# NoliNobdon/TriStage-RAG

Measured on AMD Instinct MI355X. Metric: end-to-end queries/sec @10Mx768 corpus (stage-1 exact top-k, pre-encoded HBM-resident queries), higher is better.
Workload: dtype f16; 1 GPU; synthetic 10000000x768 f16 corpus, batch-64 queries, stage-1 exact top-1000, row-sharded over 1 GPU(s); rows=10000000, dim=768, batch=64, k=1000, submission=batches enqueued back to back (async), verified by finish() in the timed region, max_candidates_per_query=6027

## Files before the change

### tristage-rag_amd/csrc/ts_scan.hip

```cpp
#include "ts_scan_dev.h"
#include "ts_linear_dev.h"
#include <stdlib.h>

template <int DT, int QH, int MODE>
__global__ __launch_bounds__(SCAN_THREADS) void scan_kernel(ScanParams p) {
  extern __shared__ __attribute__((aligned(16))) unsigned char smem[];
  u32x4* qlds = reinterpret_cast<u32x4*>(smem);
  const int tid = threadIdx.x;
  const int lane = tid & 63;
  const int wave = tid >> 6;
  const int kg = p.kg;

  const int64_t nwaves = (int64_t)gridDim.x * SCAN_WAVES;
  int64_t w = (int64_t)blockIdx.x * SCAN_WAVES + wave;
  const bool active = w < p.nwork;
  const u32x4* base = reinterpret_cast<const u32x4*>(p.corpus) + lane;
  const size_t blk_units = (size_t)kg * 64;
  int64_t blk = active ? p.blk0 + w * p.blk_stride : p.blk0;
  const u32x4* cur = base + (size_t)blk * blk_units;
  u32x4 ring[TS_RING];
  if (active) {
#pragma unroll
    for (int i = 0; i < TS_RING; ++i) ring[i] = stream_load(cur + (size_t)i * 64);
  }

  {
    const u32x4* src = reinterpret_cast<const u32x4*>(p.qimg);
    const int units = kg * QH * 64;
    for (int i0 = tid; i0 < units; i0 += 8 * SCAN_THREADS) {
      u32x4 t[8];
#pragma unroll
      for (int j = 0; j < 8; ++j) {
        const int i = i0 + j * SCAN_THREADS;
        t[j] = (i < units) ? src[i] : u32x4{0, 0, 0, 0};
      }
#pragma unroll
      for (int j = 0; j < 8; ++j) {
        const int i = i0 + j * SCAN_THREADS;
        if (i < units) qlds[i] = t[j];
      }
    }
  }
  StageLds* st = reinterpret_cast<StageLds*>(smem + (size_t)kg * QH * 1024);
  if constexpr (MODE == SCAN_FILTER) {
    if (tid == 0) st->cnt = 0;
  }
  __syncthreads();

  if (active) {

  float tau[QH];
  if constexpr (MODE == SCAN_FILTER) {
#pragma unroll
    for (int hq = 0; hq < QH; ++hq) tau[hq] = p.tau[hq * 32 + (lane & 31)];
  }

  const u32x4* ql = qlds + lane;

  while (true) {
    const int64_t wn = w + nwaves;
    const bool has_next = wn < p.nwork;
    const int64_t blkn = has_next ? (p.blk0 + wn * p.blk_stride) : blk;
    const u32x4* nxt = base + (size_t)blkn * blk_units;

    f32x16 acc[QH];
#pragma unroll
    for (int hq = 0; hq < QH; ++hq)
#pragma unroll
      for (int r = 0; r < 16; ++r) acc[hq][r] = 0.f;

    int g0 = 0;
    for (; g0 < kg - TS_RING; g0 += TS_RING) {
#pragma unroll
      for (int i = 0; i < TS_RING; ++i) {
#pragma unroll
        for (int hq = 0; hq < QH; ++hq) {
#if defined(TS_TUNING) && defined(DBG_NO_LDS)
          const u32x4 b = ring[(i + 1) % TS_RING];
#else
          const u32x4 b = ql[(size_t)((g0 + i) * QH + hq) * 64];
#endif
          mma_group<DT>(acc[hq], ring[i], b);
        }
        ring[i] = stream_load(cur + (size_t)(g0 + i + TS_RING) * 64);
        __builtin_amdgcn_sched_barrier(0);
      }
    }
#pragma unroll
    for (int i = 0; i < TS_RING; ++i) {
#pragma unroll
      for (int hq = 0; hq < QH; ++hq) {
#if defined(TS_TUNING) && defined(DBG_NO_LDS)
        const u32x4 b = ring[(i + 1) % TS_RING];
#else
        const u32x4 b = ql[(size_t)((g0 + i) * QH + hq) * 64];
#endif
        mma_group<DT>(acc[hq], ring[i], b);
      }
      ring[i] = stream_load(nxt + (size_t)i * 64);
      __builtin_amdgcn_sched_barrier(0);
    }

    if constexpr (MODE == SCAN_DENSE)
      epilogue_dense<QH>(p, acc, w, blk, lane);
    else
      epilogue_filter<QH>(p, st, acc, tau, blk, lane);

    if (!has_next) break;
    w = wn;
    blk = blkn;
    cur = nxt;
  }
  }
  if constexpr (MODE == SCAN_FILTER) flush_stage(p, st, tid);
}

typedef const uint32_t __attribute__((address_space(4)))* ts_sgpr_u32p;
typedef const int32_t __attribute__((address_space(4)))* ts_sgpr_i32p;

template <int DT, int QH>
__global__ __launch_bounds__(SCAN_THREADS) void scan_masked_kernel(MaskedScanParams p) {
  extern __shared__ __attribute__((aligned(16))) unsigned char smem[];
  u32x4* qlds = reinterpret_cast<u32x4*>(smem);
  const int tid = threadIdx.x;
  const int lane = tid & 63;
  const int wave = __builtin_amdgcn_readfirstlane(tid >> 6);
  const int kg = p.kg;

  const int64_t nwaves = (int64_t)gridDim.x * SCAN_WAVES;
  int64_t w = (int64_t)blockIdx.x * SCAN_WAVES + wave;
  const int64_t nwork = (int64_t)*(ts_sgpr_u32p)p.nlive;
  const bool active = w < nwork;
  const u32x4* base = reinterpret_cast<const u32x4*>(p.corpus) + lane;
  const size_t blk_units = (size_t)kg * 64;
  int64_t blk = active ? (int64_t)((ts_sgpr_i32p)p.live)[w] : 0;
  const u32x4* cur = base + (size_t)blk * blk_units;
  u32x4 ring[TS_RING];
  if (active) {
#pragma unroll
    for (int i = 0; i < TS_RING; ++i) ring[i] = stream_load(cur + (size_t)i * 64);
  }

  {
    const u32x4* src = reinterpret_cast<const u32x4*>(p.qimg);
    const int units = kg * QH * 64;
    for (int i0 = tid; i0 < units; i0 += 8 * SCAN_THREADS) {
      u32x4 t[8];
#pragma unroll
      for (int j = 0; j < 8; ++j) {
        const int i = i0 + j * SCAN_THREADS;
        t[j] = (i < units) ? src[i] : u32x4{0, 0, 0, 0};
      }
#pragma unroll
      for (int j = 0; j < 8; ++j) {
        const int i = i0 + j * SCAN_THREADS;
        if (i < units) qlds[i] = t[j];
      }
    }
  }
  StageLds* st = reinterpret_cast<StageLds*>(smem + (size_t)kg * QH * 1024);
  if (tid == 0) st->cnt = 0;
  __syncthreads();

  if (active) {

  float tau[QH];
  const uint32_t* mrow[QH];
  int64_t mstep[QH];
  uint32_t mor[QH], mw[QH];
#pragma unroll
  for (int hq = 0; hq < QH; ++hq) {
    tau[hq] = p.tau[hq * 32 + (lane & 31)];
    const int32_t qm = p.qmask[hq * 32 + (lane & 31)];
    mrow[hq] = p.allow_bits + (qm < 0 ? 0 : (int64_t)qm * p.allow_words);
    mstep[hq] = qm < 0 ? 0 : 1;
    mor[hq] = qm < 0 ? ~0u : 0u;
    mw[hq] = mrow[hq][blk * mstep[hq]] | mor[hq];
  }

  const u32x4* ql = qlds + lane;

  while (true) {
    const int64_t wn = w + nwaves;
    const bool has_next = wn < nwork;
    const int64_t blkn = has_next ? (int64_t)((ts_sgpr_i32p)p.live)[wn] : blk;
    const u32x4* nxt = base + (size_t)blkn * blk_units;

    f32x16 acc[QH];
#pragma unroll
    for (int hq = 0; hq < QH; ++hq)
#pragma unroll
      for (int r = 0; r < 16; ++r) acc[hq][r] = 0.f;

    int g0 = 0;
    for (; g0 < kg - TS_RING; g0 += TS_RING) {
#pragma unroll
      for (int i = 0; i < TS_RING; ++i) {
#pragma unroll
        for (int hq = 0; hq < QH; ++hq) {
          const u32x4 b = ql[(size_t)((g0 + i) * QH + hq) * 64];
          mma_group<DT>(acc[hq], ring[i], b);
        }
        ring[i] = stream_load(cur + (size_t)(g0 + i + TS_RING) * 64);
        __builtin_amdgcn_sched_barrier(0);
      }
    }
    uint32_t mwn[QH];
#pragma unroll
    for (int hq = 0; hq < QH; ++hq) mwn[hq] = mrow[hq][blkn * mstep[hq]];
#pragma unroll
    for (int i = 0; i < TS_RING; ++i) {
#pragma unroll
      for (int hq = 0; hq < QH; ++hq) {
        const u32x4 b = ql[(size_t)((g0 + i) * QH + hq) * 64];
        mma_group<DT>(acc[hq], ring[i], b);
      }
      ring[i] = stream_load(nxt + (size_t)i * 64);
      __builtin_amdgcn_sched_barrier(0);
    }

    epilogue_filter<QH, StageLds, true>(p, st, acc, tau, blk, lane, mw);

    if (!has_next) break;
    w = wn;
    blk = blkn;
    cur = nxt;
#pragma unroll
    for (int hq = 0; hq < QH; ++hq) mw[hq] = mwn[hq] | mor[hq];
  }
  }
  flush_stage(p, st, tid);
}

struct StageMultiHdr {
  uint32_t cnt;
  uint32_t pad[3];
  uint32_t qcnt[TS_MAX_GROUPS * 32];
  uint32_t qbase[TS_MAX_GROUPS * 32];
  uint32_t qoff[TS_MAX_GROUPS * 32];
};
static_assert(SCAN_WAVES <= 8 && TS_MAX_GROUPS * 32 <= 128, "survivor key fields");
#define TS_MULTI_MAX_ITERS (1 << 17)
#define TS_MULTI_MIN_STAGE 1024u
#define TS_MULTI_MAX_STAGE 4096u

template <int G, class T, int N>
__device__ __forceinline__ T pick_group(const T (&a)[N], int g) {
  T r = a[0];
#pragma unroll
  for (int i = 1; i < G; ++i) r = (g == i) ? a[i] : r;
  return r;
}

template <int G, int QB, bool TOMB, class P, class H>
__device__ __forceinline__ void epilogue_multi(const P& p, H* st, float* sscore,
                                               uint32_t* skey, const f32x16 (&acc)[G], const float (&tau)[G],
                                               int64_t blk, uint32_t keyhi, int lane) {
#if defined(TS_TUNING) && defined(DBG_EPILOGUE_MASKS)
  bool hit = false;
#pragma unroll
  for (int hq = 0; hq < G; ++hq) hit |= (acc_max(acc[hq]) >= tau[hq]);
  if (__builtin_amdgcn_ballot_w64(hit) == 0ull) return;
  const int64_t row_base = blk * TS_ROWS_PER_BLOCK;
  const int j = lane & 31;
#pragma unroll
  for (int hq = 0; hq < G; ++hq) {
    uint32_t mask = 0;
#pragma unroll
    for (int r = 0; r < 16; ++r) {
      const bool ok = (acc[hq][r] >= tau[hq]) && (row_base + acc_row(r, lane) < p.ntotal);
      mask |= ok ? (1u << r) : 0u;
    }
    if (mask) {
      uint32_t slot = atomicAdd(&st->cnt, (uint32_t)__builtin_popcount(mask));
#pragma unroll
      for (int r = 0; r < 16; ++r) {
        if (mask & (1u << r)) {
          if (slot < p.stage_cap) {
            sscore[slot] = acc[hq][r];
            skey[slot] = keyhi | ((uint32_t)acc_row(r, lane) << QB) | (uint32_t)(hq * 32 + j);
          } else {
            if constexpr (TOMB) {
              atomicMax(&p.gcnt[hq][j], p.cand_cap + 1u);
            } else {
              const uint32_t g = atomicAdd(&p.gcnt[hq][j], 1u);
              if (g < p.cand_cap) {
                p.gscore[hq][(size_t)j * p.cand_cap + g] = acc[hq][r];
                p.gid[hq][(size_t)j * p.cand_cap + g] = (int32_t)(row_base + acc_row(r, lane));
              }
            }
          }
          ++slot;
        }
      }
    }
  }
#else
  uint64_t gm[G], any = 0;
#pragma unroll
  for (int hq = 0; hq < G; ++hq) {
    gm[hq] = __builtin_amdgcn_ballot_w64(acc_max(acc[hq]) >= tau[hq]);
    any |= gm[hq];
  }
  if (any == 0ull) return;
  const int64_t row_base = blk * TS_ROWS_PER_BLOCK;
  const bool partial = row_base + TS_ROWS_PER_BLOCK > p.ntotal;
  const int rows_left = (int)(p.ntotal - row_base);
#pragma unroll
  for (int hq = 0; hq < G; ++hq) {
    if (gm[hq] == 0ull) continue;
#pragma unroll
    for (int r = 0; r < 16; ++r) {
      const bool ok = acc[hq][r] >= tau[hq];
      if (__builtin_expect(__builtin_amdgcn_ballot_w64(ok) == 0ull, 1)) continue;
      if (!ok) continue;
      int ln = lane;
      __asm__ volatile("" : "+v"(ln));
      const int row = acc_row(r, ln), j = ln & 31;
      if (!partial || row < rows_left) {
        const uint32_t slot = atomicAdd(&st->cnt, 1u);
        if (slot < p.stage_cap) {
          sscore[slot] = acc[hq][r];
          skey[slot] = keyhi | ((uint32_t)row << QB) | (uint32_t)(hq * 32 + j);
        } else {
          if constexpr (TOMB) {
            atomicMax(&p.gcnt[hq][j], p.cand_cap + 1u);
          } else {
            const uint32_t g = atomicAdd(&p.gcnt[hq][j], 1u);
            if (g < p.cand_cap) {
              p.gscore[hq][(size_t)j * p.cand_cap + g] = acc[hq][r];
              p.gid[hq][(size_t)j * p.cand_cap + g] = (int32_t)(row_base + row);
            }
          }
        }
      }
    }
  }
#endif
}

template <bool TOMB, class P>
__device__ __forceinline__ bool tomb_live(const P& p, int64_t row) {
  if constexpr (TOMB) return (p.live[row >> 5] >> (row & 31)) & 1u;
  return true;
}

template <int DT, int G, bool TOMB>
__global__ __launch_bounds__(SCAN_THREADS) void scan_multi_kernel(
    std::conditional_t<TOMB, MultiTombParams, MultiScanParams> p) {
  extern __shared__ __attribute__((aligned(16))) unsigned char smem[];
  u32x4* qlds = reinterpret_cast<u32x4*>(smem);
  const int tid = threadIdx.x;
  const int lane = tid & 63;
  const int wave = __builtin_amdgcn_readfirstlane(tid >> 6);
  const int kg = p.kg;

  const int64_t nwaves = (int64_t)gridDim.x * SCAN_WAVES;
  int64_t w = (int64_t)blockIdx.x * SCAN_WAVES + wave;
  const bool active = w < p.nwork;
  const u32x4* base = reinterpret_cast<const u32x4*>(p.corpus) + lane;
  const size_t blk_units = (size_t)kg * 64;
  int64_t blk = active ? p.blk0 + w * p.blk_stride : p.blk0;
  const u32x4* cur = base + (size_t)blk * blk_units;
  u32x4 ring[TS_RING];
  if (active) {
#pragma unroll
    for (int i = 0; i < TS_RING; ++i) ring[i] = stream_load(cur + (size_t)i * 64);
  }

  {
    const int units = kg * G * 64;
    for (int i0 = tid; i0 < units; i0 += 8 * SCAN_THREADS) {
      u32x4 t[8];
#pragma unroll
      for (int jj = 0; jj < 8; ++jj) {
        const int i = i0 + jj * SCAN_THREADS;
        t[jj] = u32x4{0, 0, 0, 0};
        if (i < units) {
          const int u = i >> 6, gk = u / G, g = u - gk * G;
          const u32x4* src = reinterpret_cast<const u32x4*>(pick_group<G>(p.gimg, g));
          t[jj] = src[(size_t)(gk * pick_group<G>(p.gqh, g) + pick_group<G>(p.ghalf, g)) * 64 + (i & 63)];
        }
      }
#pragma unroll
      for (int jj = 0; jj < 8; ++jj) {
        const int i = i0 + jj * SCAN_THREADS;
        if (i < units) qlds[i] = t[jj];
      }
    }
  }
  StageMultiHdr* st = reinterpret_cast<StageMultiHdr*>(smem + (size_t)kg * G * 1024);
  float* sscore = reinterpret_cast<float*>(st + 1);
  uint32_t* skey = reinterpret_cast<uint32_t*>(sscore + p.stage_cap);
  if (tid == 0) st->cnt = 0;
  __syncthreads();

  if (active) {

  float tau[G];
#pragma unroll
  for (int hq = 0; hq < G; ++hq) tau[hq] = p.gtau[hq][lane & 31];

  const u32x4* ql = qlds + lane;
  uint32_t keyhi = (uint32_t)wave << 12;

  while (true) {
    const int64_t wn = w + nwaves;
    const bool has_next = wn < p.nwork;
    const int64_t blkn = has_next ? (p.blk0 + wn * p.blk_stride) : blk;
    const u32x4* nxt = base + (size_t)blkn * blk_units;

    f32x16 acc[G];
#pragma unroll
    for (int hq = 0; hq < G; ++hq)
#pragma unroll
      for (int r = 0; r < 16; ++r) acc[hq][r] = 0.f;

    int g0 = 0;
    for (; g0 < kg - TS_RING; g0 += TS_RING) {
#pragma unroll
      for (int i = 0; i < TS_RING; ++i) {
#pragma unroll
        for (int hq = 0; hq < G; ++hq) {
          const u32x4 b = ql[(size_t)((g0 + i) * G + hq) * 64];
          mma_group<DT>(acc[hq], ring[i], b);
        }
        ring[i] = stream_load(cur + (size_t)(g0 + i + TS_RING) * 64);
        __builtin_amdgcn_sched_barrier(0);
      }
    }
#pragma unroll
    for (int i = 0; i < TS_RING; ++i) {
#pragma unroll
      for (int hq = 0; hq < G; ++hq) {
        const u32x4 b = ql[(size_t)((g0 + i) * G + hq) * 64];
        mma_group<DT>(acc[hq], ring[i], b);
      }
      ring[i] = stream_load(nxt + (size_t)i * 64);
      __builtin_amdgcn_sched_barrier(0);
    }

    epilogue_multi<G, 7, TOMB>(p, st, sscore, skey, acc, tau, blk, keyhi, lane);

    if (!has_next) break;
    w = wn;
    blk = blkn;
    cur = nxt;
    keyhi += 1u << 15;
  }
  }

  __syncthreads();
  const uint32_t n = st->cnt < p.stage_cap ? st->cnt : p.stage_cap;
  if (n == 0) return;
  if (tid < G * 32) { st->qcnt[tid] = 0; st->qoff[tid] = 0; }
  __syncthreads();
  auto key_row = [&](uint32_t key) {
    const int64_t wi = (int64_t)blockIdx.x * SCAN_WAVES + ((key >> 12) & 7u) + (int64_t)(key >> 15) * nwaves;
    return (p.blk0 + wi * p.blk_stride) * TS_ROWS_PER_BLOCK + ((key >> 7) & 31u);
  };
  for (uint32_t e = tid; e < n; e += SCAN_THREADS) {
    if constexpr (TOMB)
      if (!tomb_live<TOMB>(p, key_row(skey[e]))) continue;
    atomicAdd(&st->qcnt[skey[e] & 127u], 1u);
  }
  __syncthreads();
  if (tid < G * 32 && st->qcnt[tid] > 0)
    st->qbase[tid] = atomicAdd(pick_group<G>(p.gcnt, tid >> 5) + (tid & 31), st->qcnt[tid]);
  __syncthreads();
  for (uint32_t e = tid; e < n; e += SCAN_THREADS) {
    const uint32_t key = skey[e];
    if constexpr (TOMB)
      if (!tomb_live<TOMB>(p, key_row(key))) continue;
    const uint32_t q = key & 127u;
    const uint32_t slot = st->qbase[q] + atomicAdd(&st->qoff[q], 1u);
    if (slot < p.cand_cap) {
      const int g = (int)(q >> 5);
      const size_t at = (size_t)(q & 31u) * p.cand_cap + slot;
      const int64_t wi = (int64_t)blockIdx.x * SCAN_WAVES + ((key >> 12) & 7u) + (int64_t)(key >> 15) * nwaves;
      pick_group<G>(p.gscore, g)[at] = sscore[e];
      pick_group<G>(p.gid, g)[at] = (int32_t)((p.blk0 + wi * p.blk_stride) * TS_ROWS_PER_BLOCK + ((key >> 7) & 31u));
    }
  }
}

int ts_scan_multi_groups(const TsLayout& L) {
  if (L.dtype != TS_F16 && L.dtype != TS_BF16) return 0;
  for (int G = TS_MAX_GROUPS; G >= 1; --G)
    if (ts_scan_multi_stage_cap(L, G) > 0) return G;
  return 0;
}

uint32_t ts_scan_multi_stage_cap(const TsLayout& L, int G) {
  const size_t fixed = (size_t)L.kg * G * 1024 + sizeof(StageMultiHdr);
  if (G < 1 || G > TS_MAX_GROUPS || fixed + 8 * (size_t)TS_MULTI_MIN_STAGE > 160 * 1024) return 0;
  return (uint32_t)std::min<size_t>(TS_MULTI_MAX_STAGE, (160 * 1024 - fixed) / 8);
}

bool ts_scan_multi_fits(int64_t nblk, int num_cus) {
  const int64_t want = (nblk + SCAN_WAVES - 1) / SCAN_WAVES;
  const int64_t grid = std::max<int64_t>(1, std::min<int64_t>(want, num_cus));
  const int64_t nwaves = grid * SCAN_WAVES;
  return (nblk + nwaves - 1) / nwaves <= TS_MULTI_MAX_ITERS;
}

template <int DT, int G, class P = MultiScanParams>
static int launch_scan_multi_t(const TsLayout& L, const P& p, int num_cus, hipStream_t stream) {
  const size_t lds = (size_t)L.kg * G * 1024 + sizeof(StageMultiHdr) + 8 * (size_t)p.stage_cap;
  void (*kern)(P) = scan_multi_kernel<DT, G, std::is_same<P, MultiTombParams>::value>;
  static TsDeviceOnce lds_attr;
  TS_CHECK(ts_allow_max_lds(lds_attr, reinterpret_cast<const void*>(kern)));
  const int64_t want = (p.nwork + SCAN_WAVES - 1) / SCAN_WAVES;
  int grid = (int)(want < num_cus ? want : num_cus);
  if (grid < 1) grid = 1;
  hipLaunchKernelGGL(kern, dim3(grid), dim3(SCAN_THREADS), lds, stream, p);
  TS_HIP(hipGetLastError());
  return TS_OK;
}

template <class P>
static int launch_scan_multi_any(const TsLayout& L, int G, const P& p, int num_cus, hipStream_t stream) {
  if (p.nwork <= 0) return TS_OK;
  if (p.stage_cap == 0 || p.stage_cap > ts_scan_multi_stage_cap(L, G) || !ts_scan_multi_fits(p.nwork, num_cus)) {
    ts_set_error("multi-group scan: %d groups do not fit at dimension %d", G, L.dim);
    return TS_ERR_UNSUPPORTED;
  }
#define TS_MULTI_G(DT)                                                      \
  switch (G) {                                                              \
    case 1: return launch_scan_multi_t<DT, 1, P>(L, p, num_cus, stream);    \
    case 2: return launch_scan_multi_t<DT, 2, P>(L, p, num_cus, stream);    \
    case 3: return launch_scan_multi_t<DT, 3, P>(L, p, num_cus, stream);    \
    case 4: return launch_scan_multi_t<DT, 4, P>(L, p, num_cus, stream);    \
  }
  switch (L.dtype) {
    case TS_F16: TS_MULTI_G(TS_F16); break;
    case TS_BF16: TS_MULTI_G(TS_BF16); break;
  }
#undef TS_MULTI_G
  ts_set_error("multi-group scan: bad dtype %d or group count %d", L.dtype, G);
  return TS_ERR_UNSUPPORTED;
}

int ts_launch_scan_multi(const TsLayout& L, int G, const MultiScanParams& p, int num_cus, hipStream_t stream) {
  return launch_scan_multi_any(L, G, p, num_cus, stream);
}

int ts_launch_scan_multi_tomb(const TsLayout& L, int G, const MultiTombParams& p, int num_cus, hipStream_t stream) {
  return launch_scan_multi_any(L, G, p, num_cus, stream);
}

struct StageWideHdr {
  uint32_t cnt;
  uint32_t pad[3];
  uint32_t qcnt[TS_MAX_WIDE_GROUPS * 32];
  uint32_t qbase[TS_MAX_WIDE_GROUPS * 32];
  uint32_t qoff[TS_MAX_WIDE_GROUPS * 32];
};
static_assert(SCAN_WAVES <= 8 && TS_MAX_WIDE_GROUPS * 32 <= 256, "wide survivor key fields");
static_assert(SCAN_THREADS == TS_RING * 64, "a window is G units per thread");
#define TS_WIDE_GROUPS 6
#define TS_WIDE_MAX_ITERS (1 << 16)
#define TS_WIDE_MIN_STAGE 4096u
#define TS_WIDE_MAX_STAGE 8192u

template <int N, int I = 0, class F>
__device__ __forceinline__ void ts_static_for(F&& f) {
  if constexpr (I < N) {
    f(std::integral_constant<int, I>{});
    ts_static_for<N, I + 1>(f);
  }
}

template <int I>
__device__ __forceinline__ void wide_ring_load(u32x4& r, uint32_t loff, const unsigned char* fill) {
#if defined(TS_TUNING) && defined(DBG_NO_MFMA)
  r = stream_load(reinterpret_cast<const u32x4*>(fill + loff + I * 1024));
#else
  __asm__ volatile("s_nop 4\n\tglobal_load_dwordx4 %0, %1, %2 offset:%3 nt"
                   : "=v"(r) : "v"(loff), "s"(fill + (I / 4) * 4096), "i"((I % 4) * 1024) : "memory");
#endif
}

#if defined(TS_TUNING) && defined(WIDE_TRACE)
#define WIDE_TRACE_ROW 10
__device__ uint32_t wide_trace_buf[256 * SCAN_WAVES * WIDE_TRACE_ROW];
extern "C" int ts_debug_wide_trace(uint32_t* out) {
  return hipMemcpyFromSymbol(out, HIP_SYMBOL(wide_trace_buf), sizeof(wide_trace_buf)) == hipSuccess ? 0 : -2;
}
#define WIDE_TRACE_BEGIN()                                              \
  uint32_t wt_sum[6] = {0, 0, 0, 0, 0, 0};                              \
  const uint32_t wt_c0 = (uint32_t)__builtin_readcyclecounter();        \
  const uint32_t wt_t0 = (uint32_t)__builtin_amdgcn_s_memrealtime();    \
  uint32_t wt_last = wt_t0
#define WIDE_STAMP(k)                                                   \
  do {                                                                  \
    __builtin_amdgcn_sched_barrier(0);                                  \
    const uint32_t now_ = (uint32_t)__builtin_amdgcn_s_memrealtime();   \
    wt_sum[k] += now_ - wt_last;                                        \
    wt_last = now_;                                                     \
    __builtin_amdgcn_sched_barrier(0);                                  \
  } while (0)
#define WIDE_STAMP_READS(k)                                             \
  do {                                                                  \
    __builtin_amdgcn_sched_barrier(0);                                  \
    __builtin_amdgcn_s_waitcnt(0xC07F);                 \
    WIDE_STAMP(k);                                                      \
  } while (0)
#define WIDE_TRACE_END(nwindows)                                                                     \
  do {                                                                                               \
    if (lane == 0 && blockIdx.x < 256) {                                                             \
      uint32_t* row_ = wide_trace_buf + ((size_t)blockIdx.x * SCAN_WAVES + wave) * WIDE_TRACE_ROW;   \
      for (int k_ = 0; k_ < 6; ++k_) row_[k_] = wt_sum[k_];                                          \
      row_[6] = (uint32_t)__builtin_amdgcn_s_memrealtime() - wt_t0;                                  \
      row_[7] = (uint32_t)__builtin_readcyclecounter() - wt_c0;                                      \
      row_[8] = (uint32_t)(nwindows);                                                                \
    }                                                                                                \
  } while (0)
#else
#define WIDE_TRACE_BEGIN() do { } while (0)
#define WIDE_STAMP(k) do { } while (0)
#define WIDE_STAMP_READS(k) do { } while (0)
#define WIDE_TRACE_END(nwindows) do { } while (0)
#endif

#if defined(TS_TUNING) && defined(DBG_WIDE_STAGGER)
#define TS_WIDE_STAGGER DBG_WIDE_STAGGER
#else
#define TS_WIDE_STAGGER (-1)
#endif
static_assert(TS_WIDE_STAGGER >= -1 && TS_WIDE_STAGGER < TS_RING - 1, "stagger slots");

template <int DT, int G, bool TOMB>
__global__ __launch_bounds__(SCAN_THREADS) void scan_wide_kernel(
    std::conditional_t<TOMB, WideTombParams, WideScanParams> p) {
  extern __shared__ __attribute__((aligned(16))) unsigned char smem[];
  constexpr int WU = G * TS_RING * 64;
  u32x4* win = reinterpret_cast<u32x4*>(smem);
  const int tid = threadIdx.x;
  const int lane = tid & 63;
  const int wave = __builtin_amdgcn_readfirstlane(tid >> 6);
  const int kg = p.kg;
  const int nwin = kg / TS_RING;

  const int64_t nwaves = (int64_t)gridDim.x * SCAN_WAVES;
  const int64_t w0 = (int64_t)blockIdx.x * SCAN_WAVES;
  int64_t w = w0 + wave;
  const bool active = w < p.nwork;
  const size_t blk_units = (size_t)kg * 64;
  int64_t blk = active ? p.blk0 + w * p.blk_stride : p.blk0;

  const int64_t my_iters = active ? (p.nwork - 1 - w) / nwaves + 1 : 0;
  const int64_t wg_iters = w0 < p.nwork ? (p.nwork - 1 - w0) / nwaves + 1 : 0;
  const int64_t tw_mine = my_iters * nwin, tw_all = wg_iters * nwin;

  const unsigned char* corpus = reinterpret_cast<const unsigned char*>(p.corpus);
  const uint32_t loff = (uint32_t)lane * 16;
  int64_t fw = w;
  const unsigned char* fill = corpus + (size_t)blk * blk_units * 16;
  const unsigned char* const fill_dead = reinterpret_cast<const unsigned char*>(p.gimg[0]);
  bool fill_done = false;
  int fwin = 0;
  auto advance_fill = [&]() {
    if (fill_done) return;
    if (++fwin < nwin) {
      fill += TS_RING * 1024;
    } else if (fw + nwaves < p.nwork) {
      fwin = 0;
      fw += nwaves;
      fill = corpus + (size_t)(p.blk0 + fw * p.blk_stride) * blk_units * 16;
    } else {
      fill_done = true;
      fill = fill_dead;
    }
  };
#if defined(TS_TUNING) && defined(DBG_WIDE_L2_RING)
  fill = fill_dead;
  fill_done = true;
#endif
  auto refill = [&](u32x4& r, auto slot) { wide_ring_load<decltype(slot)::value>(r, loff, fill); };
  auto ring_wait = [&](u32x4& r, auto slot) {
    constexpr int I = decltype(slot)::value;
    __asm__ volatile("s_waitcnt vmcnt(%1)" : "+v"(r)
                     : "i"(I <= TS_WIDE_STAGGER ? 2 * TS_RING - 1 + G - I : 2 * TS_RING - 1 + 2 * G));
  };

  const unsigned char* qsrc[G];
  int64_t qstep[G];
#pragma unroll
  for (int j = 0; j < G; ++j) {
    const int v = wave + SCAN_WAVES * j, i = v / G, g = v - i * G;
    const int gqh = pick_group<G>(p.gqh, g);
    qsrc[j] = reinterpret_cast<const unsigned char*>(pick_group<G>(p.gimg, g)) +
              (size_t)(i * gqh + pick_group<G>(p.ghalf, g)) * 1024;
    qstep[j] = (int64_t)gqh * TS_RING * 1024;
  }
  const uint32_t win_lds = (uint32_t)(uintptr_t)(__attribute__((address_space(3))) void*)(win + wave * 64);
  auto gather = [&](int wi, int b) {
#pragma unroll
    for (int j = 0; j < G; ++j) {
      const unsigned char* src = qsrc[j] + wi * qstep[j];
      const uint32_t dst = win_lds + (uint32_t)(b * WU + j * SCAN_THREADS) * 16;
      uint32_t keep;
      __asm__ volatile("s_nop 4\n\ts_mov_b32 %0, m0\n\ts_mov_b32 m0, %3\n\ts_nop 0\n\t"
                       "global_load_lds_dwordx4 %1, %2\n\ts_mov_b32 m0, %0"
                       : "=&s"(keep) : "v"(loff), "s"(src), "s"(dst) : "memory");
    }
  };

  StageWideHdr* st = reinterpret_cast<StageWideHdr*>(smem + (size_t)2 * WU * 16);
  float* sscore = reinterpret_cast<float*>(st + 1);
  uint32_t* skey = reinterpret_cast<uint32_t*>(sscore + p.stage_cap);
  if (tid == 0) st->cnt = 0;

  float tau[G];
#pragma unroll
  for (int hq = 0; hq < G; ++hq) tau[hq] = p.gtau[hq][lane & 31];
#pragma unroll
  for (int hq = 0; hq < G; ++hq) __asm__ volatile("" : "+v"(tau[hq]));
  u32x4 ring[2 * TS_RING];
  if (active) {
    ts_static_for<TS_RING>([&](auto i) { refill(ring[i], i); });
    advance_fill();
  }
  gather(0, 0);
  if (active) {
    ts_static_for<TS_RING>([&](auto i) { refill(ring[TS_RING + i], i); });
    advance_fill();
    __builtin_amdgcn_s_waitcnt(0x3F70 | TS_RING);
  } else {
    __builtin_amdgcn_s_waitcnt(0x3F70);
  }
  fs_barrier();

  uint32_t keyhi = (uint32_t)wave << 13;

  f32x16 acc[G];
#pragma unroll
  for (int hq = 0; hq < G; ++hq)
#pragma unroll
    for (int r = 0; r < 16; ++r) acc[hq][r] = 0.f;

  auto walk_barrier = [&]() {
#if defined(TS_TUNING) && defined(DBG_WIDE_NO_BARRIER)
    __builtin_amdgcn_s_waitcnt(0xC07F);
#else
    fs_barrier();
#endif
  };
  int qw = 0;
  WIDE_TRACE_BEGIN();
  auto window = [&](auto half) {
    constexpr int P = decltype(half)::value;
    const int qn = qw + 1 < nwin ? qw + 1 : 0;
    __builtin_amdgcn_s_waitcnt(0xC07F);
    const bool late = TS_WIDE_STAGGER >= 0 && wave >= SCAN_WAVES / 2;
    if (!late) gather(qn, P ^ 1);
    WIDE_STAMP(0);
    const u32x4* ql = win + P * WU + lane;
#if !(defined(TS_TUNING) && defined(DBG_WIDE_SERIAL_B))
    u32x4 bb[G];
#pragma unroll
    for (int hq = 0; hq < G; ++hq) bb[hq] = ql[hq * 64];
#endif
    WIDE_STAMP_READS(1);
    ts_static_for<TS_RING>([&](auto i) {
#if defined(TS_TUNING) && defined(DBG_WIDE_SERIAL_B)
      ring_wait(ring[P * TS_RING + i], i);
#pragma unroll
      for (int hq = 0; hq < G; ++hq) {
        const u32x4 b = ql[(i * G + hq) * 64];
        mma_group<DT>(acc[hq], ring[P * TS_RING + i], b);
      }
#else
      __builtin_amdgcn_sched_barrier(0);
      ring_wait(ring[P * TS_RING + i], i);
#pragma unroll
      for (int hq = 0; hq < G; ++hq) {
        mma_group<DT>(acc[hq], ring[P * TS_RING + i], bb[hq]);
        __builtin_amdgcn_sched_barrier(0);
        if constexpr (decltype(i)::value + 1 < TS_RING) {
          bb[hq] = ql[((i + 1) * G + hq) * 64];
          __builtin_amdgcn_sched_barrier(0);
        }
      }
#endif
      if constexpr (decltype(i)::value == TS_WIDE_STAGGER) {
        if (late) gather(qn, P ^ 1);
        ts_static_for<TS_WIDE_STAGGER + 1>([&](auto k) { refill(ring[P * TS_RING + k], k); });
      } else if constexpr (decltype(i)::value > TS_WIDE_STAGGER) {
        refill(ring[P * TS_RING + i], i);
      }
      __builtin_amdgcn_sched_barrier(0);
    });
    WIDE_STAMP(2);
    advance_fill();
    if (qw == nwin - 1) {
      epilogue_multi<G, 8, TOMB>(p, st, sscore, skey, acc, tau, blk, keyhi, lane);
#pragma unroll
      for (int hq = 0; hq < G; ++hq)
#pragma unroll
        for (int r = 0; r < 16; ++r) acc[hq][r] = 0.f;
      w += nwaves;
      blk = p.blk0 + w * p.blk_stride;
      keyhi += 1u << 16;
    }
    WIDE_STAMP(3);
    __builtin_amdgcn_s_waitcnt(0x3F70 | TS_RING);
    WIDE_STAMP(4);
    walk_barrier();
    WIDE_STAMP(5);
    qw = qn;
  };
  int64_t t = 0;
  for (; t < tw_mine; t += 2) {
    window(std::integral_constant<int, 0>{});
    if (t + 1 == tw_mine) { ++t; break; }
    window(std::integral_constant<int, 1>{});
  }
  __builtin_amdgcn_s_waitcnt(0x3F70);
  for (; t < tw_all; ++t) {
    const int qn = qw + 1 < nwin ? qw + 1 : 0;
    gather(qn, (int)(t & 1) ^ 1);
    __builtin_amdgcn_s_waitcnt(0x3F70);
    walk_barrier();
    qw = qn;
  }
  WIDE_TRACE_END(tw_mine);

  __syncthreads();
  const uint32_t n = st->cnt < p.stage_cap ? st->cnt : p.stage_cap;
  if (n == 0) return;
  for (int t = tid; t < G * 32; t += SCAN_THREADS) { st->qcnt[t] = 0; st->qoff[t] = 0; }
  __syncthreads();
  auto key_row = [&](uint32_t key) {
    const int64_t wi = (int64_t)blockIdx.x * SCAN_WAVES + ((key >> 13) & 7u) + (int64_t)(key >> 16) * nwaves;
    return (p.blk0 + wi * p.blk_stride) * TS_ROWS_PER_BLOCK + ((key >> 8) & 31u);
  };
  for (uint32_t e = tid; e < n; e += SCAN_THREADS) {
    if constexpr (TOMB)
      if (!tomb_live<TOMB>(p, key_row(skey[e]))) continue;
    atomicAdd(&st->qcnt[skey[e] & 255u], 1u);
  }
  __syncthreads();
  for (int t = tid; t < G * 32; t += SCAN_THREADS)
    if (st->qcnt[t] > 0) st->qbase[t] = atomicAdd(pick_group<G>(p.gcnt, t >> 5) + (t & 31), st->qcnt[t]);
  __syncthreads();
  for (uint32_t e = tid; e < n; e += SCAN_THREADS) {
    const uint32_t key = skey[e];
    if constexpr (TOMB)
      if (!tomb_live<TOMB>(p, key_row(key))) continue;
    const uint32_t q = key & 255u;
    const uint32_t slot = st->qbase[q] + atomicAdd(&st->qoff[q], 1u);
    if (slot < p.cand_cap) {
      const int g = (int)(q >> 5);
      const size_t at = (size_t)(q & 31u) * p.cand_cap + slot;
      const int64_t wi = (int64_t)blockIdx.x * SCAN_WAVES + ((key >> 13) & 7u) + (int64_t)(key >> 16) * nwaves;
      pick_group<G>(p.gscore, g)[at] = sscore[e];
      pick_group<G>(p.gid, g)[at] = (int32_t)((p.blk0 + wi * p.blk_stride) * TS_ROWS_PER_BLOCK + ((key >> 8) & 31u));
    }
  }
}

int ts_scan_wide_groups(const TsLayout& L) {
  if (L.dtype != TS_F16 && L.dtype != TS_BF16) return 0;
  return ts_scan_wide_stage_cap(L, TS_WIDE_GROUPS) > 0 ? TS_WIDE_GROUPS : 0;
}

uint32_t ts_scan_wide_stage_cap(const TsLayout& L, int G) {
  (void)L;
  const size_t fixed = (size_t)2 * G * TS_RING * 1024 + sizeof(StageWideHdr);
  if (G < 2 || G > TS_WIDE_GROUPS || fixed + 8 * (size_t)TS_WIDE_MIN_STAGE > 160 * 1024) return 0;
  return (uint32_t)std::min<size_t>(TS_WIDE_MAX_STAGE, (160 * 1024 - fixed) / 8);
}

bool ts_scan_wide_fits(int64_t nblk, int num_cus) {
  const int64_t want = (nblk + SCAN_WAVES - 1) / SCAN_WAVES;
  const int64_t grid = std::max<int64_t>(1, std::min<int64_t>(want, num_cus));
  const int64_t nwaves = grid * SCAN_WAVES;
  return (nblk + nwaves - 1) / nwaves <= TS_WIDE_MAX_ITERS;
}

template <int DT, int G, class P = WideScanParams>
static int launch_scan_wide_t(const P& p, int num_cus, hipStream_t stream) {
  const size_t lds = (size_t)2 * G * TS_RING * 1024 + sizeof(StageWideHdr) + 8 * (size_t)p.stage_cap;
  void (*kern)(P) = scan_wide_kernel<DT, G, std::is_same<P, WideTombParams>::value>;
  static TsDeviceOnce lds_attr;
  TS_CHECK(ts_allow_max_lds(lds_attr, reinterpret_cast<const void*>(kern)));
  const int64_t want = (p.nwork + SCAN_WAVES - 1) / SCAN_WAVES;
  int grid = (int)(want < num_cus ? want : num_cus);
  if (grid < 1) grid = 1;
  hipLaunchKernelGGL(kern, dim3(grid), dim3(SCAN_THREADS), lds, stream, p);
  TS_HIP(hipGetLastError());
  return TS_OK;
}

template <class P>
static int launch_scan_wide_any(const TsLayout& L, int G, const P& p, int num_cus, hipStream_t stream) {
  if (p.nwork <= 0) return TS_OK;
  if (p.stage_cap == 0 || p.stage_cap > ts_scan_wide_stage_cap(L, G) || !ts_scan_wide_fits(p.nwork, num_cus) ||
      L.kg % TS_RING != 0) {
    ts_set_error("wide scan: %d groups do not fit at dimension %d", G, L.dim);
    return TS_ERR_UNSUPPORTED;
  }
#define TS_WIDE_G(DT)                                                   \
  switch (G) {                                                          \
    case 2: return launch_scan_wide_t<DT, 2, P>(p, num_cus, stream);    \
    case 3: return launch_scan_wide_t<DT, 3, P>(p, num_cus, stream);    \
    case 4: return launch_scan_wide_t<DT, 4, P>(p, num_cus, stream);    \
    case 5: return launch_scan_wide_t<DT, 5, P>(p, num_cus, stream);    \
    case 6: return launch_scan_wide_t<DT, 6, P>(p, num_cus, stream);    \
  }
  switch (L.dtype) {
    case TS_F16: TS_WIDE_G(TS_F16); break;
    case TS_BF16: TS_WIDE_G(TS_BF16); break;
  }
#undef TS_WIDE_G
  ts_set_error("wide scan: bad dtype %d or group count %d", L.dtype, G);
  return TS_ERR_UNSUPPORTED;
}

int ts_launch_scan_wide(const TsLayout& L, int G, const WideScanParams& p, int num_cus, hipStream_t stream) {
  return launch_scan_wide_any(L, G, p, num_cus, stream);
}

int ts_launch_scan_wide_tomb(const TsLayout& L, int G, const WideTombParams& p, int num_cus, hipStream_t stream) {
  return launch_scan_wide_any(L, G, p, num_cus, stream);
}

bool ts_use_f32_split(const TsLayout& L, int qh) {
  if (L.dtype != TS_F32 || qh != 1) return false;
#ifdef TS_TUNING
  static const bool off = getenv("TS_NO_F32_SPLIT") != nullptr;
  if (off) return false;
#endif
  const size_t s = ts_scan_f32s_lds_bytes(L);
  if (s == 0 || s > 160 * 1024) return false;
  return (size_t)L.kg * 2 * 1024 + sizeof(StageLds) > 160 * 1024;
}

size_t ts_scan_lds_bytes(const TsLayout& L, int qh) {
  if (L.dtype == TS_FP8_E4M3) return ts_scan_fp8_lds_bytes(L, qh);
  if (ts_use_f32_split(L, qh)) return ts_scan_f32s_lds_bytes(L);
  return (size_t)L.kg * qh * 1024 + sizeof(StageLds);
}

template <int DT, int QH, int MODE>
static int launch_scan_t(const TsLayout& L, const ScanParams& p, int num_cus,
                         hipStream_t stream) {
  const size_t lds = (size_t)L.kg * QH * 1024 + (MODE == SCAN_FILTER ? sizeof(StageLds) : 0);
  auto kern = scan_kernel<DT, QH, MODE>;
  static TsDeviceOnce lds_attr;
  TS_CHECK(ts_allow_max_lds(lds_attr, reinterpret_cast<const void*>(kern)));
  int wg_per_cu = 1;
  if (MODE == SCAN_DENSE && 2 * lds <= 160 * 1024) wg_per_cu = 2;
  int64_t want = (p.nwork + SCAN_WAVES - 1) / SCAN_WAVES;
  int64_t cap = (int64_t)num_cus * wg_per_cu;
  int grid = (int)(want < cap ? want : cap);
  if (grid < 1) grid = 1;
  hipLaunchKernelGGL(kern, dim3(grid), dim3(SCAN_THREADS), lds, stream, p);
  TS_HIP(hipGetLastError());
  return TS_OK;
}

template <int DT, int QH>
static int launch_scan_masked_t(const TsLayout& L, const MaskedScanParams& p, int num_cus, hipStream_t stream) {
  const size_t lds = (size_t)L.kg * QH * 1024 + sizeof(StageLds);
  auto kern = scan_masked_kernel<DT, QH>;
  static TsDeviceOnce lds_attr;
  TS_CHECK(ts_allow_max_lds(lds_attr, reinterpret_cast<const void*>(kern)));
  int64_t want = (p.nwork + SCAN_WAVES - 1) / SCAN_WAVES;
  int grid = (int)(want < num_cus ? want : num_cus);
  if (grid < 1) grid = 1;
  hipLaunchKernelGGL(kern, dim3(grid), dim3(SCAN_THREADS), lds, stream, p);
  TS_HIP(hipGetLastError());
  return TS_OK;
}

int ts_launch_scan_masked(const TsLayout& L, int qh, const MaskedScanParams& p, int num_cus, hipStream_t stream) {
  if (p.nwork <= 0) return TS_OK;
  if (L.dtype == TS_FP8_E4M3) return ts_launch_scan_masked_fp8(L, qh, p, num_cus, stream);
  if (ts_scan_lds_bytes(L, qh) > 160 * 1024) {
    ts_set_error("dimension %d too large for the LDS-resident query image", L.dim);
    return TS_ERR_UNSUPPORTED;
  }
  switch (L.dtype) {
    case TS_F16: return qh == 1 ? launch_scan_masked_t<TS_F16, 1>(L, p, num_cus, stream)
                                : launch_scan_masked_t<TS_F16, 2>(L, p, num_cus, stream);
    case TS_BF16: return qh == 1 ? launch_scan_masked_t<TS_BF16, 1>(L, p, num_cus, stream)
                                 : launch_scan_masked_t<TS_BF16, 2>(L, p, num_cus, stream);
  }
  ts_set_error("the masked scan takes f16 / bf16 storage only");
  return TS_ERR_UNSUPPORTED;
}

template <int DT>
static int launch_scan_dt(const TsLayout& L, int mode, int qh,
                          const ScanParams& p, int num_cus, hipStream_t s) {
  if (qh == 1) {
    return mode == SCAN_DENSE ? launch_scan_t<DT, 1, SCAN_DENSE>(L, p, num_cus, s)
                              : launch_scan_t<DT, 1, SCAN_FILTER>(L, p, num_cus, s);
  }
  return mode == SCAN_DENSE ? launch_scan_t<DT, 2, SCAN_DENSE>(L, p, num_cus, s)
                            : launch_scan_t<DT, 2, SCAN_FILTER>(L, p, num_cus, s);
}

int ts_launch_scan(const TsLayout& L, int mode, int qh, const ScanParams& p,
                   int num_cus, hipStream_t stream) {
  if (p.nwork <= 0) return TS_OK;
  if (L.dtype == TS_FP8_E4M3) return ts_launch_scan_fp8(L, mode, qh, p, num_cus, stream);
  if (ts_use_f32_split(L, qh)) return ts_launch_scan_f32s(L, mode, p, num_cus, stream);
  if (ts_scan_lds_bytes(L, qh) > 160 * 1024) {
    ts_set_error("dimension %d too large for the LDS-resident query image", L.dim);
    return TS_ERR_UNSUPPORTED;
  }
  switch (L.dtype) {
    case TS_F16: return launch_scan_dt<TS_F16>(L, mode, qh, p, num_cus, stream);
    case TS_BF16: return launch_scan_dt<TS_BF16>(L, mode, qh, p, num_cus, stream);
    case TS_F32: return launch_scan_dt<TS_F32>(L, mode, qh, p, num_cus, stream);
  }
  ts_set_error("bad dtype %d", L.dtype);
  return TS_ERR_INVALID;
}

__global__ __launch_bounds__(256) void live_blocks_kernel(const uint32_t* bits, int64_t words, TsMaskPass mp,
                                                          int64_t nblk, int64_t ntotal, TsMaskDev* md) {
  const int tid = threadIdx.x;
  const int lane = tid & 63;
  if (blockIdx.x == 0 && tid < TS_MAX_Q) {
    md->qmask[tid] = mp.qmask[tid];
    md->qd[tid] = mp.qd[tid];
  }
  const int64_t b = (int64_t)blockIdx.x * blockDim.x + tid;
  const bool in = b < nblk;
  const int64_t rows = in ? ntotal - b * TS_ROWS_PER_BLOCK : 0;
  const uint32_t valid = rows >= 32 ? ~0u : (rows > 0 ? ((1u << rows) - 1u) : 0u);
  uint32_t any = 0;
  for (int d = 0; d < mp.nd; ++d) {
    const uint32_t wd = in ? (bits[(int64_t)mp.dist[d] * words + b] & valid) : 0u;
    any |= wd;
    uint32_t c = (uint32_t)__builtin_popcount(wd);
#pragma unroll
    for (int off = 32; off > 0; off >>= 1) c += (uint32_t)__shfl_xor((int)c, off, 64);
    if (lane == 0 && c) atomicAdd(&md->popc[d], c);
  }
  if (mp.all_live) any = valid;
  const bool live = any != 0u;
  const unsigned long long bal = __builtin_amdgcn_ballot_w64(live);
  if (bal == 0ull) return;
  uint32_t base = 0;
  if (lane == 0) base = atomicAdd(&md->nlive, (uint32_t)__builtin_popcountll(bal));
  base = (uint32_t)__shfl((int)base, 0, 64);
  if (live) {
    const uint32_t below = (uint32_t)__builtin_popcountll(bal & ((1ull << lane) - 1ull));
    reinterpret_cast<int32_t*>(md + 1)[base + below] = (int32_t)b;
  }
}

int ts_launch_live_blocks(const uint32_t* bits, int64_t words, const TsMaskPass& mp, int64_t nblk,
                          int64_t ntotal, TsMaskDev* md, hipStream_t stream) {
  const int64_t blocks = (nblk + 255) / 256;
  if (blocks < 1 || blocks > 0x7fffffffLL) { ts_set_error("live blocks: bad row block count"); return TS_ERR_INVALID; }
  hipLaunchKernelGGL(live_blocks_kernel, dim3((unsigned)blocks), dim3(256), 0, stream, bits, words, mp, nblk, ntotal, md);
  TS_HIP(hipGetLastError());
  return TS_OK;
}

template <typename TIN>
__global__ void row_den_kernel(const TIN* rows, int64_t n, int dim, float* den) {
  const int lane = threadIdx.x & 63;
  const int64_t row = (int64_t)blockIdx.x * (blockDim.x >> 6) + (threadIdx.x >> 6);
  if (row >= n) return;
  const TIN* src = rows + row * dim;
  float s = 0.f;
  for (int k = lane; k < dim; k += 64) {
    float v = ElemIO<TIN>::ld(src + k);
    s += v * v;
  }
#pragma unroll
  for (int off = 32; off > 0; off >>= 1) s += __shfl_xor(s, off, 64);
  if (lane == 0) den[row] = sqrtf(s) + 1e-8f;
}

template <typename TIN>
__global__ void relayout_kernel(const TIN* rows, int64_t n, int dim,
                                int64_t row0, int64_t blk_first, int64_t nunits_wave,
                                uint4* tiled, int kg, int dt, const float* den, int vec) {
  const int lane = threadIdx.x & 63;
  const int64_t wv = (int64_t)blockIdx.x * (blockDim.x >> 6) + (threadIdx.x >> 6);
  if (wv >= nunits_wave) return;
  const int64_t b = blk_first + wv / kg;
  const int g = (int)(wv % kg);
  const int r = lane & 31, h = lane >> 5;
  const int64_t row = b * TS_ROWS_PER_BLOCK + r;
  if (row < row0 || row >= row0 + n) return;
  const TIN* src = rows + (row - row0) * dim;
  const float d = den ? den[row - row0] : 1.0f;
  u32x4 out;
  if (dt == TS_F32) {
#pragma unroll
    for (int e = 0; e < 4; ++e) {
      const int k = frag_k(dt, g, h, e);
      float v = (k < dim) ? ElemIO<TIN>::ld(src + k) : 0.f;
      if (den) v = v / d;
      out[e] = __builtin_bit_cast(uint32_t, v);
    }
  } else if (vec) {
    const int k0 = frag_k(dt, g, h, 0);
    float v[8];
    if (k0 < dim) {
      ld8<TIN>(src + k0, v);
    } else {
#pragma unroll
      for (int e = 0; e < 8; ++e) v[e] = 0.f;
    }
#pragma unroll
    for (int e = 0; e < 4; ++e) {
      float v0 = v[2 * e], v1 = v[2 * e + 1];
      if (den) { v0 = v0 / d; v1 = v1 / d; }
      out[e] = (uint32_t)f32_to_storage16(v0, dt) | ((uint32_t)f32_to_storage16(v1, dt) << 16);
    }
  } else {
#pragma unroll
    for (int e = 0; e < 4; ++e) {
      const int k0 = frag_k(dt, g, h, 2 * e), k1 = k0 + 1;
      float v0 = (k0 < dim) ? ElemIO<TIN>::ld(src + k0) : 0.f;
      float v1 = (k1 < dim) ? ElemIO<TIN>::ld(src + k1) : 0.f;
      if (den) { v0 = v0 / d; v1 = v1 / d; }
      out[e] = (uint32_t)f32_to_storage16(v0, dt) |
               ((uint32_t)f32_to_storage16(v1, dt) << 16);
    }
  }
  reinterpret_cast<u32x4*>(tiled)[(size_t)(b * kg + g) * 64 + lane] = out;
}

int ts_launch_row_den(const void* rows, int in_dtype, int64_t n, int dim, float* den, hipStream_t s) {
  const int blocks = (int)((n + 3) / 4);
  switch (in_dtype) {
    case TS_F32: hipLaunchKernelGGL(row_den_kernel<float>, dim3(blocks), dim3(256), 0, s, (const float*)rows, n, dim, den); break;
    case TS_F16: hipLaunchKernelGGL(row_den_kernel<_Float16>, dim3(blocks), dim3(256), 0, s, (const _Float16*)rows, n, dim, den); break;
    case TS_BF16: hipLaunchKernelGGL(row_den_kernel<__bf16>, dim3(blocks), dim3(256), 0, s, (const __bf16*)rows, n, dim, den); break;
    default: ts_set_error("bad rows dtype %d", in_dtype); return TS_ERR_INVALID;
  }
  TS_HIP(hipGetLastError());
  return TS_OK;
}

template <typename TIN>
static int relayout_t(const TsLayout& L, const TIN* rows, int64_t n, int64_t row0,
                      uint4* tiled, bool normalize, float* den, hipStream_t s) {
  if (normalize) {
    int blocks = (int)((n + 3) / 4);
    hipLaunchKernelGGL(row_den_kernel<TIN>, dim3(blocks), dim3(256), 0, s, rows, n,
                       L.dim, den);
    TS_HIP(hipGetLastError());
  }
  const int64_t blk_first = row0 / TS_ROWS_PER_BLOCK;
  const int64_t blk_last = (row0 + n - 1) / TS_ROWS_PER_BLOCK;
  const int64_t nwave = (blk_last - blk_first + 1) * L.kg;
  const int64_t blocks = (nwave + 3) / 4;
  if (blocks > 0x7fffffffLL) {
    ts_set_error("add: too many rows in one call");
    return TS_ERR_INVALID;
  }
  hipLaunchKernelGGL(relayout_kernel<TIN>, dim3((unsigned)blocks), dim3(256), 0, s,
                     rows, n, L.dim, row0, blk_first, nwave, tiled, L.kg, L.dtype,
                     normalize ? den : (const float*)nullptr,
                     (int)(L.dtype != TS_F32 && (L.dim % 8) == 0 &&
                           (reinterpret_cast<uintptr_t>(rows) % (4 * sizeof(TIN) >= 16 ? 32 : 16)) == 0));
  TS_HIP(hipGetLastError());
  return TS_OK;
}

int ts_launch_relayout(const TsLayout& L, const void* rows, int in_dtype, int64_t n,
                       int64_t row0, uint4* tiled, bool normalize,
                       float* den_scratch, hipStream_t stream) {
  if (n <= 0) return TS_OK;
  if (L.dtype == TS_FP8_E4M3)
    return ts_launch_relayout_fp8(L, rows, in_dtype, n, row0, tiled, normalize, den_scratch, stream);
  switch (in_dtype) {
    case TS_F32: return relayout_t<float>(L, (const float*)rows, n, row0, tiled, normalize, den_scratch, stream);
    case TS_F16: return relayout_t<_Float16>(L, (const _Float16*)rows, n, row0, tiled, normalize, den_scratch, stream);
    case TS_BF16: return relayout_t<__bf16>(L, (const __bf16*)rows, n, row0, tiled, normalize, den_scratch, stream);
  }
  ts_set_error("bad rows dtype %d", in_dtype);
  return TS_ERR_INVALID;
}

__global__ void reconstruct_kernel(const uint4* tiled, int64_t row0, int64_t n,
                                   int dim, int kg, int dt, float* out) {
  const int upr = kg * 2;
  const int64_t t = (int64_t)blockIdx.x * blockDim.x + threadIdx.x;
  if (t >= n * upr) return;
  const int64_t row = row0 + t / upr;
  const int u = (int)(t % upr);
  const int g = u >> 1, h = u & 1;
  const int64_t b = row / TS_ROWS_PER_BLOCK;
  const int lane = h * 32 + (int)(row % TS_ROWS_PER_BLOCK);
  const u32x4 v = reinterpret_cast<const u32x4*>(tiled)[(size_t)(b * kg + g) * 64 + lane];
  float* dst = out + (row - row0) * dim;
  if (dt == TS_F32) {
#pragma unroll
    for (int e = 0; e < 4; ++e) {
      const int k = frag_k(dt, g, h, e);
      const uint32_t w = v[e];
      if (k < dim) dst[k] = __uint_as_float(w);
    }
  } else {
#pragma unroll
    for (int e = 0; e < 8; ++e) {
      const int k = frag_k(dt, g, h, e);
      const uint16_t bits = (uint16_t)(v[e >> 1] >> (16 * (e & 1)));
      float f;
      if (dt == TS_F16) f = (float)__builtin_bit_cast(_Float16, bits);
      else f = __builtin_bit_cast(float, (uint32_t)bits << 16);
      if (k < dim) dst[k] = f;
    }
  }
}

int ts_launch_reconstruct(const TsLayout& L, const uint4* tiled, int64_t row0,
                          int64_t n, float* out, hipStream_t stream) {
  if (n <= 0) return TS_OK;
  if (L.dtype == TS_FP8_E4M3) return ts_launch_reconstruct_fp8(L, tiled, row0, n, out, stream);
  const int64_t total = n * L.kg * 2;
  const int64_t blocks = (total + 255) / 256;
  if (blocks > 0x7fffffffLL) {
    ts_set_error("reconstruct: range too large");
    return TS_ERR_INVALID;
  }
  hipLaunchKernelGGL(reconstruct_kernel, dim3((unsigned)blocks), dim3(256), 0, stream,
                     tiled, row0, n, L.dim, L.kg, L.dtype, out);
  TS_HIP(hipGetLastError());
  return TS_OK;
}

template <typename TIN>
__global__ void qprep_kernel(const TIN* q, int nq, int dim, int kg, int qh, int dt,
                             uint4* qimg, uint32_t* cand_cnt, uint32_t* status) {
  const int t = blockIdx.x * blockDim.x + threadIdx.x;
  if (t < TS_MAX_Q && cand_cnt) cand_cnt[t] = 0;
  if (t == 0 && status) status[0] = 0;
  if (t >= kg * qh * 64) return;
  const int lane = t & 63;
  const int hq = (t >> 6) % qh;
  const int g = (t >> 6) / qh;
  const int j = lane & 31, h = lane >> 5;
  const int qi = hq * 32 + j;
  const TIN* src = q + (int64_t)qi * dim;
  u32x4 out;
  if (dt == TS_F32) {
#pragma unroll
    for (int e = 0; e < 4; ++e) {
      const int k = frag_k(dt, g, h, e);
      float v = (qi < nq && k < dim) ? ElemIO<TIN>::ld(src + k) : 0.f;
      out[e] = __builtin_bit_cast(uint32_t, v);
    }
  } else {
#pragma unroll
    for (int e = 0; e < 4; ++e) {
      const int k0 = frag_k(dt, g, h, 2 * e), k1 = k0 + 1;
      float v0 = (qi < nq && k0 < dim) ? ElemIO<TIN>::ld(src + k0) : 0.f;
      float v1 = (qi < nq && k1 < dim) ? ElemIO<TIN>::ld(src + k1) : 0.f;
      out[e] = (uint32_t)f32_to_storage16(v0, dt) |
               ((uint32_t)f32_to_storage16(v1, dt) << 16);
    }
  }
  reinterpret_cast<u32x4*>(qimg)[t] = out;
}

int ts_launch_qprep(const TsLayout& L, const void* q, int q_dtype, int nq, int qh,
                    uint4* qimg, uint32_t* cand_cnt, uint32_t* status,
                    hipStream_t stream) {
  if (L.dtype == TS_FP8_E4M3) return ts_launch_qprep_fp8(L, q, q_dtype, nq, qh, qimg, cand_cnt, status, stream);
  if (ts_use_f32_split(L, qh)) return ts_launch_qprep_f32s(L, q, q_dtype, nq, qimg, cand_cnt, status, stream);
  const int units = L.kg * qh * 64;
  const int blocks = (units + 255) / 256;
  switch (q_dtype) {
    case TS_F32:
      hipLaunchKernelGGL(qprep_kernel<float>, dim3(blocks), dim3(256), 0, stream,
                         (const float*)q, nq, L.dim, L.kg, qh, L.dtype, qimg, cand_cnt, status);
      break;
    case TS_F16:
      hipLaunchKernelGGL(qprep_kernel<_Float16>, dim3(blocks), dim3(256), 0, stream,
                         (const _Float16*)q, nq, L.dim, L.kg, qh, L.dtype, qimg, cand_cnt, status);
      break;
    case TS_BF16:
      hipLaunchKernelGGL(qprep_kernel<__bf16>, dim3(blocks), dim3(256), 0, stream,
                         (const __bf16*)q, nq, L.dim, L.kg, qh, L.dtype, qimg, cand_cnt, status);
      break;
    default:
      ts_set_error("bad query dtype %d", q_dtype);
      return TS_ERR_INVALID;
  }
  TS_HIP(hipGetLastError());
  return TS_OK;
}
```

Before: 56560 queries/s.

## Allow half of waves to load query windows; drop stagger debug path

```diff
diff --git a/tristage-rag_amd/csrc/ts_scan.hip b/tristage-rag_amd/csrc/ts_scan.hip
--- a/tristage-rag_amd/csrc/ts_scan.hip
+++ b/tristage-rag_amd/csrc/ts_scan.hip
@@ -614,6 +614,7 @@
       row_[6] = (uint32_t)__builtin_amdgcn_s_memrealtime() - wt_t0;                                  \
       row_[7] = (uint32_t)__builtin_readcyclecounter() - wt_c0;                                      \
       row_[8] = (uint32_t)(nwindows);                                                                \
+      row_[9] = TS_WIDE_LOADERS < 0 ? 0u : loader ? 2u : 1u;                                         \
     }                                                                                                \
   } while (0)
 #else
@@ -623,12 +624,12 @@
 #define WIDE_TRACE_END(nwindows) do { } while (0)
 #endif
 
-#if defined(TS_TUNING) && defined(DBG_WIDE_STAGGER)
-#define TS_WIDE_STAGGER DBG_WIDE_STAGGER
-#else
-#define TS_WIDE_STAGGER (-1)
+#ifndef TS_WIDE_LOADERS
+#define TS_WIDE_LOADERS (-1)
 #endif
-static_assert(TS_WIDE_STAGGER >= -1 && TS_WIDE_STAGGER < TS_RING - 1, "stagger slots");
+static_assert(TS_WIDE_LOADERS >= -1 && TS_WIDE_LOADERS <= 1, "which half of a workgroup's waves loads");
+#define TS_WIDE_NLOAD (TS_WIDE_LOADERS < 0 ? SCAN_WAVES : SCAN_WAVES / 2)
+static_assert(SCAN_WAVES == 8 && TS_RING * 8 % TS_WIDE_NLOAD == 0, "a loader's share of a window");
 
 template <int DT, int G, bool TOMB>
 __global__ __launch_bounds__(SCAN_THREADS) void scan_wide_kernel(
@@ -677,33 +678,42 @@
   fill = fill_dead;
   fill_done = true;
 #endif
+  constexpr int NL = TS_WIDE_NLOAD;
+  constexpr int QP = G * TS_RING / NL;
+  const bool loader = TS_WIDE_LOADERS < 0 || (wave < SCAN_WAVES / 2) == (TS_WIDE_LOADERS == 0);
   auto refill = [&](u32x4& r, auto slot) { wide_ring_load<decltype(slot)::value>(r, loff, fill); };
-  auto ring_wait = [&](u32x4& r, auto slot) {
-    constexpr int I = decltype(slot)::value;
-    __asm__ volatile("s_waitcnt vmcnt(%1)" : "+v"(r)
-                     : "i"(I <= TS_WIDE_STAGGER ? 2 * TS_RING - 1 + G - I : 2 * TS_RING - 1 + 2 * G));
+  auto ring_wait = [&](u32x4& r) {
+    if (loader) {
+      __asm__ volatile("s_waitcnt vmcnt(%0)" : : "i"(2 * TS_RING - 1 + 2 * QP));
+    } else {
+      __asm__ volatile("s_waitcnt vmcnt(%0)" : : "i"(2 * TS_RING - 1));
+    }
+    __asm__ volatile("" : "+v"(r));
   };
 
+  const int lr = wave & (NL - 1);
   const unsigned char* qsrc[G];
-  int64_t qstep[G];
+  uint32_t qstep[G];
 #pragma unroll
   for (int j = 0; j < G; ++j) {
-    const int v = wave + SCAN_WAVES * j, i = v / G, g = v - i * G;
+    const int v = lr + NL * j, i = v / G, g = v - i * G;
     const int gqh = pick_group<G>(p.gqh, g);
     qsrc[j] = reinterpret_cast<const unsigned char*>(pick_group<G>(p.gimg, g)) +
               (size_t)(i * gqh + pick_group<G>(p.ghalf, g)) * 1024;
-    qstep[j] = (int64_t)gqh * TS_RING * 1024;
-  }
-  const uint32_t win_lds = (uint32_t)(uintptr_t)(__attribute__((address_space(3))) void*)(win + wave * 64);
-  auto gather = [&](int wi, int b) {
-#pragma unroll
-    for (int j = 0; j < G; ++j) {
-      const unsigned char* src = qsrc[j] + wi * qstep[j];
-      const uint32_t dst = win_lds + (uint32_t)(b * WU + j * SCAN_THREADS) * 16;
+    qstep[j] = (uint32_t)gqh * TS_RING * 1024;
+  }
+  const uint32_t win_lds = (uint32_t)(uintptr_t)(__attribute__((address_space(3))) void*)(win + lr * 64);
+  auto gather = [&](int wi, auto b) {
+    const uint32_t lo = loff, base = win_lds;
+#pragma unroll
+    for (int j = 0; j < QP; ++j) {
+      const unsigned char* src = qsrc[j % G] + ((uint32_t)wi * qstep[j % G] + (j / G) * (qstep[j % G] / (TS_RING / NL)));
       uint32_t keep;
-      __asm__ volatile("s_nop 4\n\ts_mov_b32 %0, m0\n\ts_mov_b32 m0, %3\n\ts_nop 0\n\t"
+      __asm__ volatile("s_nop 4\n\ts_mov_b32 %0, m0\n\ts_add_u32 m0, %3, %4\n\ts_nop 0\n\t"
                        "global_load_lds_dwordx4 %1, %2\n\ts_mov_b32 m0, %0"
-                       : "=&s"(keep) : "v"(loff), "s"(src), "s"(dst) : "memory");
+                       : "=&s"(keep)
+                       : "v"(lo), "s"(src), "s"(base), "i"((decltype(b)::value * WU + j * NL * 64) * 16)
+                       : "memory", "scc");
     }
   };
 
@@ -722,13 +732,17 @@
     ts_static_for<TS_RING>([&](auto i) { refill(ring[i], i); });
     advance_fill();
   }
-  gather(0, 0);
+  if (loader) gather(0, std::integral_constant<int, 0>{});
   if (active) {
     ts_static_for<TS_RING>([&](auto i) { refill(ring[TS_RING + i], i); });
     advance_fill();
-    __builtin_amdgcn_s_waitcnt(0x3F70 | TS_RING);
-  } else {
-    __builtin_amdgcn_s_waitcnt(0x3F70);
+  }
+  if (loader) {
+    if (active) {
+      __builtin_amdgcn_s_waitcnt(0x3F70 | TS_RING);
+    } else {
+      __builtin_amdgcn_s_waitcnt(0x3F70);
+    }
   }
   fs_barrier();
 
@@ -753,8 +767,7 @@
     constexpr int P = decltype(half)::value;
     const int qn = qw + 1 < nwin ? qw + 1 : 0;
     __builtin_amdgcn_s_waitcnt(0xC07F);
-    const bool late = TS_WIDE_STAGGER >= 0 && wave >= SCAN_WAVES / 2;
-    if (!late) gather(qn, P ^ 1);
+    if (loader) gather(qn, std::integral_constant<int, P ^ 1>{});
     WIDE_STAMP(0);
     const u32x4* ql = win + P * WU + lane;
 #if !(defined(TS_TUNING) && defined(DBG_WIDE_SERIAL_B))
@@ -765,7 +778,7 @@
     WIDE_STAMP_READS(1);
     ts_static_for<TS_RING>([&](auto i) {
 #if defined(TS_TUNING) && defined(DBG_WIDE_SERIAL_B)
-      ring_wait(ring[P * TS_RING + i], i);
+      ring_wait(ring[P * TS_RING + i]);
 #pragma unroll
       for (int hq = 0; hq < G; ++hq) {
         const u32x4 b = ql[(i * G + hq) * 64];
@@ -773,7 +786,7 @@
       }
 #else
       __builtin_amdgcn_sched_barrier(0);
-      ring_wait(ring[P * TS_RING + i], i);
+      ring_wait(ring[P * TS_RING + i]);
 #pragma unroll
       for (int hq = 0; hq < G; ++hq) {
         mma_group<DT>(acc[hq], ring[P * TS_RING + i], bb[hq]);
@@ -784,12 +797,7 @@
         }
       }
 #endif
-      if constexpr (decltype(i)::value == TS_WIDE_STAGGER) {
-        if (late) gather(qn, P ^ 1);
-        ts_static_for<TS_WIDE_STAGGER + 1>([&](auto k) { refill(ring[P * TS_RING + k], k); });
-      } else if constexpr (decltype(i)::value > TS_WIDE_STAGGER) {
-        refill(ring[P * TS_RING + i], i);
-      }
+      refill(ring[P * TS_RING + i], i);
       __builtin_amdgcn_sched_barrier(0);
     });
     WIDE_STAMP(2);
@@ -805,7 +813,7 @@
       keyhi += 1u << 16;
     }
     WIDE_STAMP(3);
-    __builtin_amdgcn_s_waitcnt(0x3F70 | TS_RING);
+    if (loader) __builtin_amdgcn_s_waitcnt(0x3F70 | TS_RING);
     WIDE_STAMP(4);
     walk_barrier();
     WIDE_STAMP(5);
@@ -820,8 +828,14 @@
   __builtin_amdgcn_s_waitcnt(0x3F70);
   for (; t < tw_all; ++t) {
     const int qn = qw + 1 < nwin ? qw + 1 : 0;
-    gather(qn, (int)(t & 1) ^ 1);
-    __builtin_amdgcn_s_waitcnt(0x3F70);
+    if (loader) {
+      if (t & 1) {
+        gather(qn, std::integral_constant<int, 0>{});
+      } else {
+        gather(qn, std::integral_constant<int, 1>{});
+      }
+      __builtin_amdgcn_s_waitcnt(0x3F70);
+    }
     walk_barrier();
     qw = qn;
   }
```

Result: no change. 56770 queries/s, median of 6 (+0.4%).
